# zhan-xu/MoRig

Measured on AMD Instinct MI355X. Metric: meshes/sec jointnet_motion forward, 4 k-vert synthetic, higher is better.
Workload: dtype f32 (split-fp16: 3x f16 MFMA, f32 accumulate); 1 GPU; jointnet_motion(num_keyframes=5, attn) eval forward, B=64 x 4096-vertex synthetic meshes/GPU, BASELINE.json configs[1]; step=COO->CSR prep + forward, meshes_per_gpu=64, global_batch=64, vertices_per_mesh=4096, parallelism=mesh-sharded dp1, guard_read=deferred, geo_graph=device

## Files before the change

morig_amd/csrc/common.h:

```cpp
#pragma once
#include <hip/hip_runtime.h>
#include <stdint.h>
#include <string.h>
#include "../../include/morig_hip.h"
#include "ragged_core.h"

namespace morig {

enum Kind : int {
    K_GEMM_BN128 = 0, K_GEMM_BN64, K_GEMM_BN32, K_GEMM_POOL,
    K_EDGE_H16, K_EDGE_H32, K_EDGE_H64, K_EDGE_H128, K_EDGE_H256,
    K_CSR, K_COPY, K_ROWNORM, K_ATTN, K_MISC,
    K_FPS, K_BALL, K_POINTCONV, K_KNN_INTERP, K_COSINE_NN,
    K_GEMM16_BN128, K_GEMM16_BN64, K_GEMM16_BN32, K_GEMM16_POOL,
    K_EDGE16_H32, K_EDGE16_H64, K_EDGE16_H128, K_EDGE16_H256, K_POINTCONV16, K_GEMM16_DMA,
    K_COSINE_KNN, K_FLOW_VOTE, K_JOINTS,
    K_GEMM16_DMAP, K_GEMM16_DMA128, K_EDGE16_H256_PP, K_EDGE16_H128_WS, K_EDGE16_PC, K_GEOGRAPH, K_EDGE16_X3, K_EDGE_X3, K_EDGE16_X3P, K_EDGE16_H128_RL,
    K_LOSS_NCE_FWD, K_LOSS_NCE_BWD, K_LOSS_MULTIPOS, K_LOSS_CHAMFER, K_LOSS_REDUCE,
    K_LOSS_LOGRATIO, K_LOSS_SKIN_CE,
    K_METRICS,
    K_RIG_ASSEMBLE, K_RIG_ENTRIES,
    K_RANSAC_VOTE, K_RANSAC_FIT, K_RANSAC_APPLY, K_KMEANS,
    K_MESH_PREP, K_VOXEL_SURFACE, K_VOXEL_FILL,
    K_POSE_PREP, K_POSE_SKIN, K_POSE_ERRORS,
    K_SCAN_RASTER, K_SCAN,
    K_SIMPLIFY_KEYS, K_SIMPLIFY_QUADRICS,
    K_COUNT
};
static_assert(K_COUNT <= MORIG_PROF_KINDS, "raise MORIG_PROF_KINDS");

void set_hip_error(hipError_t e);
struct ProfScope {
    ProfScope(int kind, hipStream_t s, double flops, double bytes);
    ~ProfScope();
    int slot; hipStream_t stream; ProfScope* outer;
};
void prof_retag(int kind);

inline int check_hip(hipError_t e) {
    if (e == hipSuccess) return MORIG_OK;
    set_hip_error(e);
    return MORIG_E_HIP;
}
#define MORIG_HIP_TRY(expr) do { hipError_t _e = (expr); if (_e != hipSuccess) { ::morig::set_hip_error(_e); return MORIG_E_HIP; } } while (0)
#define MORIG_LAUNCH_CHECK() MORIG_HIP_TRY(hipGetLastError())

struct EdgePcParams {
    int H;
    const float* W; int ldw;
    const float* bias; const float* scale; const float* shift;
    const float* A; int lda; const float* B; int ldb;
    const int* rowptr; const int* srcS; const int* dstS; int n_nodes; int rep_in; int rep_out; int tiles_per_rep;
    int replicas;
    float* Y; int ldy;
    int y16;
    int run;
    int* ovf;
    int quad;
    int min4;
    unsigned long long* trace;
    int dbg;
};
struct GemmDmaParams {
    int M, N, K;
    const float* X; int ldx;
    const float* Xt; int ldt; int tail_rows; int tail_chunks;
    const float* W; int ldw;
    const float* bias; const float* scale; const float* shift; int relu;
    const float* rowbias; int ld_rowbias; const int* seg;
    float* Y; int ldy; int y16;
    float* pool; int ld_pool;
    int tiles_n;
    int* ovf;
    int dbg;
    unsigned long long* trace;
};
int launch_edge_pc(const EdgePcParams& p, int nblocks, hipStream_t s);
void set_reserved_cus(int n);
int reserved_cus();
int launch_edge_pp(const EdgePcParams& p, int nblocks, hipStream_t s);
int launch_edge_ws(const EdgePcParams& p, int nblocks, hipStream_t s);
int launch_edge_rl(const EdgePcParams& p, int ntiles64, hipStream_t s);
int launch_gemm16_dma(const GemmDmaParams& p, int tiles_m128, hipStream_t s);
struct EdgeX3Params {
    const float* X; int ldx;
    const float* W1a; const float* W1b; const float* b1;
    const float* A; int lda; const float* B; int ldb;
    const float* W2s; int ldw;
    const float* bias; const float* scale; const float* shift;
    const int* rowptr; const int* srcS; const int* dstS; int n_nodes; int cap;
    int rep_in, rep_out, replicas;
    float* Y; int ldy;
    int* ovf;
};

int launch_edge_x3(const EdgeX3Params& p, int n_tiles_cap, hipStream_t s);
int launch_gemm16_dmap(const GemmDmaParams& p, hipStream_t s);
bool few_rows_gemm_takes(int M, int N, int K, int ldx, int ldw);
int launch_few_rows_gemm(const float* X, int ldx, int M, const float* W, int ldw, int N, int K, const float* bias, const float* scale,
                         const float* shift, int relu, float* Y, int ldy, hipStream_t s);

static_assert(sizeof(morig_gemm_args) >= MORIG_GEMM_ARGS_V3_SIZE && sizeof(morig_edgeconv_args) >= MORIG_EDGECONV_ARGS_V3_SIZE &&
              sizeof(morig_edgeconv_x3_args) >= MORIG_EDGECONV_X3_ARGS_V3_SIZE && sizeof(morig_segmax_args) >= MORIG_SEGMAX_ARGS_V3_SIZE &&
              sizeof(morig_pointconv_args) >= MORIG_POINTCONV_ARGS_V3_SIZE, "argument structs only grow");
static_assert(sizeof(morig_edgeconv_args) == MORIG_EDGECONV_ARGS_SIZE && sizeof(morig_edgeconv_x3_args) == MORIG_EDGECONV_X3_ARGS_SIZE,
              "include/morig_hip.h states the current sizes");
template <class T> static inline bool take_args(const T* a, T& mine, uint32_t v3_size) {
    if (!a) return false;
    const uint32_t n = a->struct_size;
    if (n < v3_size || n > 1024u || (n & 7u)) return false;
    memset(&mine, 0, sizeof(T));
    memcpy(&mine, a, n < sizeof(T) ? n : sizeof(T));
    mine.struct_size = (uint32_t)sizeof(T);
    return true;
}

static inline int cdiv(long a, long b) { return (int)((a + b - 1) / b); }

__device__ __forceinline__ void atomic_max_f32(float* addr, float v) {
    if (v == 0.0f) v = 0.0f;
    if (v >= 0.0f) atomicMax(reinterpret_cast<int*>(addr), __float_as_int(v));
    else           atomicMin(reinterpret_cast<unsigned int*>(addr), __float_as_uint(v));
}

__device__ __forceinline__ int xcd_remap(int b, int n) {
    const int q = n >> 3, r = n & 7, x = b & 7, i = b >> 3;
    return (x < r ? x * (q + 1) : r * (q + 1) + (x - r) * q) + i;
}

inline int stats_slab_rows(int rows_cap, int cols) {
    const int groups = (cols + 63) / 64;
    int slabs = 1024 / (groups > 0 ? groups : 1);
    if (slabs < 64) slabs = 64;
    int r = ((rows_cap > 0 ? rows_cap : 1) + slabs - 1) / slabs;
    r = (r + 3) & ~3;
    return r < 256 ? 256 : r;
}

#ifdef __HIPCC__
__device__ inline void split_pair_f16(float v0, float v1, float& hi, float& lo) {
    typedef __fp16 split_h2 __attribute__((ext_vector_type(2)));
    const split_h2 h = __builtin_amdgcn_cvt_pkrtz(v0, v1);
    hi = __builtin_bit_cast(float, h);
#ifdef MORIG_SPLIT_C_FORM
    split_h2 l;
    l[0] = (__fp16)(v0 - (float)h[0]); l[1] = (__fp16)(v1 - (float)h[1]);
    lo = __builtin_bit_cast(float, l);
#else
    asm("v_fma_mixlo_f16 %0, %1, 1.0, -%2 op_sel_hi:[0,0,1]" : "=v"(lo) : "v"(v0), "v"(hi));
    asm("v_fma_mixhi_f16 %0, %1, 1.0, -%2 op_sel:[0,0,1] op_sel_hi:[0,0,1]" : "+v"(lo) : "v"(v1), "v"(hi));
#endif
}
#endif

#ifdef __HIPCC__
__device__ inline void split_pair_bf16(float v0, float v1, float& hi, float& lo) {
    typedef __bf16 split_b2 __attribute__((ext_vector_type(2)));
    const split_b2 h = {(__bf16)v0, (__bf16)v1};
    const unsigned hb = __builtin_bit_cast(unsigned, h);
    hi = __builtin_bit_cast(float, h);
    const float r0 = v0 - __uint_as_float(hb << 16), r1 = v1 - __uint_as_float(hb & 0xffff0000u);
    const split_b2 l = {(__bf16)r0, (__bf16)r1};
    lo = __builtin_bit_cast(float, l);
}
#endif

#ifdef __HIPCC__
__device__ inline void split_pair_bf16_rem(float v0, float v1, float& hi, float& r0, float& r1) {
    typedef __bf16 split_b2 __attribute__((ext_vector_type(2)));
    const split_b2 h = {(__bf16)v0, (__bf16)v1};
    const unsigned hb = __builtin_bit_cast(unsigned, h);
    hi = __builtin_bit_cast(float, h);
    r0 = v0 - __uint_as_float(hb << 16);
    r1 = v1 - __uint_as_float(hb & 0xffff0000u);
}
#endif

template <int V> struct VecF { float v[V]; };
#ifdef __HIPCC__
template <int V> __device__ inline VecF<V> ldv(const float* p) {
    VecF<V> r;
    if constexpr (V == 4) { const float4 t = *reinterpret_cast<const float4*>(p); r.v[0] = t.x; r.v[1] = t.y; r.v[2] = t.z; r.v[3] = t.w; }
    else r.v[0] = *p;
    return r;
}
template <int V> __device__ inline void stv(float* p, const VecF<V>& r) {
    if constexpr (V == 4) *reinterpret_cast<float4*>(p) = make_float4(r.v[0], r.v[1], r.v[2], r.v[3]);
    else *p = r.v[0];
}
#endif
static inline bool vec4_ptr(const void* p, long ld) { return (reinterpret_cast<uintptr_t>(p) & 15) == 0 && (ld & 3) == 0; }

#ifdef __HIPCC__
__device__ inline void stats_block_store(const double (&acc)[2][4], int quads, int RL, int q, int rl, int c0, int cols, int slab,
                                         double* __restrict__ part) {
    __shared__ double sh[2 * 1024];
    const int gc = quads * 4;
    if (rl < RL) {
#pragma unroll
        for (int k = 0; k < 2; ++k)
#pragma unroll
            for (int j = 0; j < 4; ++j) sh[(k * gc + q * 4 + j) * RL + rl] = acc[k][j];
    }
    __syncthreads();
    const int t = threadIdx.x;
    if (t < 2 * gc) {
        const int k = t / gc, col = t - k * gc;
        double s = 0.0;
        for (int i = 0; i < RL; ++i) s += sh[(k * gc + col) * RL + i];
        if (c0 + col < cols) part[((size_t)slab * 2 + k) * cols + c0 + col] = s;
    }
}

constexpr int STATS_FC = 4;
__device__ inline void stats_final_sums(const double* __restrict__ part, int slabs, int cols, int c, double& s, double& q) {
    const int sl = threadIdx.x / STATS_FC, l = threadIdx.x % STATS_FC;
    constexpr int LANES = 256 / STATS_FC;
    s = 0.0; q = 0.0;
    if (c < cols)
        for (int b = sl; b < slabs; b += LANES) { s += part[((size_t)b * 2 + 0) * cols + c]; q += part[((size_t)b * 2 + 1) * cols + c]; }
    __shared__ double sh[2][LANES][STATS_FC];
    sh[0][sl][l] = s; sh[1][sl][l] = q;
    __syncthreads();
    for (int h = LANES / 2; h > 0; h >>= 1) {
        if (sl < h) { sh[0][sl][l] += sh[0][sl + h][l]; sh[1][sl][l] += sh[1][sl + h][l]; }
        __syncthreads();
    }
    s = sh[0][0][l]; q = sh[1][0][l];
}

__device__ __forceinline__ double block_sum256(double s, double* sh) {
    sh[threadIdx.x] = s;
    __syncthreads();
    for (int h = 128; h > 0; h >>= 1) {
        if ((int)threadIdx.x < h) sh[threadIdx.x] += sh[threadIdx.x + h];
        __syncthreads();
    }
    const double r = sh[0];
    __syncthreads();
    return r;
}
#endif

}
```

morig_amd/csrc/gemm_dma.hip:

```cpp
#include "common.h"
#include "epilogue_store.h"
#include <stdlib.h>
#include <stdlib.h>

namespace morig {

typedef float f32x16 __attribute__((ext_vector_type(16)));
typedef _Float16 f16x8 __attribute__((ext_vector_type(8)));
typedef __attribute__((address_space(3))) void lds_void_t;
typedef __attribute__((address_space(1))) const void glb_void_t;

template <int BM, int BN, int NT, int DMA_NS, bool TR = false, bool TAIL = false>
__global__ __launch_bounds__((BM / 64) * (BN / (32 * NT)) * 64) void gemm16_dma_kernel(const GemmDmaParams p) {
    constexpr int MT = 2;
    constexpr int WNW = BN / (32 * NT);
    constexpr int NW = (BM / 64) * WNW;
    constexpr int DMA_STAGE = (BM + BN) * 128;
    constexpr int XJ = BM / 8 / NW, WJ = BN / 8 / NW;
    constexpr int PER_CHUNK = XJ + WJ;
    constexpr int TBYTES = NW * EpilogueTile<NT>::FLOATS * 4;
    constexpr int RING = DMA_NS * DMA_STAGE;
    constexpr int SM0 = (TR || RING > TBYTES) ? RING : TBYTES;
    constexpr int PANEL = TR ? 3 * BN * 4 : 0;
    __shared__ __attribute__((aligned(128))) char smem[SM0 + BM * 4 + PANEL];
    int* sseg = reinterpret_cast<int*>(smem + SM0);
    float* pan = reinterpret_cast<float*>(smem + SM0 + BM * 4);

    const int tid = threadIdx.x, lane = tid & 63, wave = tid >> 6;
    const int l31 = lane & 31, hi = lane >> 5;
    const int wm = wave / WNW, wn = wave % WNW;
    const int lin = xcd_remap(blockIdx.x, gridDim.x);
    const int tn = lin % p.tiles_n, tm = lin / p.tiles_n;
    const int row0 = tm * BM;

#ifdef MORIG_DMA_TRACE
#define DMA_TS(k) do { if ((int)blockIdx.x == (int)(gridDim.x / 2 + 8) && lane == 0) p.trace[(k) * 8 + wave] = __builtin_readcyclecounter(); } while (0)
#else
#define DMA_TS(k) do { } while (0)
#endif
    DMA_TS(0);
    if (!TR && p.seg != nullptr && tid < BM) sseg[tid] = (row0 + tid < p.M) ? p.seg[row0 + tid] : 0;
    float pv_b = 0.f, pv_s = 1.f, pv_t = 0.f;
    bool rb_slow = false;
    if constexpr (TR) {
        if (tid < BN) {
            const int col = tn * BN + tid;
            if (p.bias) pv_b = p.bias[col];
            if (p.scale) { pv_s = p.scale[col]; pv_t = p.shift[col]; }
        }
        if (p.rowbias != nullptr) {
            const int s0 = p.seg[row0], s1 = p.seg[min(row0 + BM, p.M) - 1];
            rb_slow = s0 != s1;
            if (!rb_slow && tid < BN) pv_b += p.rowbias[(size_t)s0 * p.ld_rowbias + tn * BN + tid];
        }
    }

    unsigned ox[XJ], ow[WJ];
    const int rsub = lane >> 3;
    const int pslot = lane & 7;
    const char* xbase = reinterpret_cast<const char*>(p.X + (size_t)row0 * p.ldx);
    const char* wbase = reinterpret_cast<const char*>(p.W + (size_t)(tn * BN) * p.ldw);
#pragma unroll
    for (int j = 0; j < XJ; ++j) {
        const int r = (wave * XJ + j) * 8 + rsub;
        const int lslot = pslot ^ ((r >> 1) & 7);
        int xr = r; if (row0 + xr >= p.M) xr = p.M - 1 - row0;
        ox[j] = ((unsigned)xr * (unsigned)p.ldx + 4u * lslot) * 4u;
    }
#pragma unroll
    for (int j = 0; j < WJ; ++j) {
        const int r = (wave * WJ + j) * 8 + rsub;
        ow[j] = ((unsigned)r * (unsigned)p.ldw + 4u * (pslot ^ ((r >> 1) & 7))) * 4u;
    }
    const int nchunk = (p.K + 31) / 32;
    unsigned ot[TAIL ? XJ : 1];
    const int c_tail = TAIL ? nchunk - p.tail_chunks : nchunk;
    const char* tbase = reinterpret_cast<const char*>(p.Xt);
    if constexpr (TAIL) {
#pragma unroll
        for (int j = 0; j < XJ; ++j) {
            const int r = (wave * XJ + j) * 8 + rsub;
            int gr = row0 + r; if (gr >= p.M) gr = p.M - 1;
            ot[j] = ((unsigned)(gr % p.tail_rows) * (unsigned)p.ldt + 4u * (unsigned)(pslot ^ ((r >> 1) & 7))) * 4u;
        }
    }
    auto x_src = [&](int c, int j) __attribute__((always_inline)) -> const char* {
        unsigned o = ox[j];
        const char* b = xbase + c * 128;
        if constexpr (TAIL) { if (c >= c_tail) { o = ot[j]; b = tbase + (c - c_tail) * 128; } }
        asm volatile("" : "+v"(o));
        return b + o;
    };
    auto issue_x = [&](int c) {
        char* st = smem + (c % DMA_NS) * DMA_STAGE;
#pragma unroll
        for (int j = 0; j < XJ; ++j)
            __builtin_amdgcn_global_load_lds((glb_void_t*)x_src(c, j), (lds_void_t*)(st + (wave * XJ + j) * 1024), 16, 0, 0);
    };
    auto issue_w = [&](int c) {
        char* st = smem + (c % DMA_NS) * DMA_STAGE;
#pragma unroll
        for (int j = 0; j < WJ; ++j) {
            unsigned o = ow[j];
            asm volatile("" : "+v"(o));
            __builtin_amdgcn_global_load_lds((glb_void_t*)(wbase + c * 128 + o), (lds_void_t*)(st + BM * 128 + (wave * WJ + j) * 1024), 16, 0, 0);
        }
    };
    auto issue = [&](int c) { issue_x(c); issue_w(c); };

    f32x16 acc[MT][NT];
#pragma unroll
    for (int mt = 0; mt < MT; ++mt)
#pragma unroll
        for (int nt = 0; nt < NT; ++nt)
#pragma unroll
            for (int r = 0; r < 16; ++r) acc[mt][nt][r] = 0.f;

#pragma unroll
    for (int c = 0; c < DMA_NS - 1; ++c) if (c < nchunk) issue(c);
    if constexpr (TR) { if (tid < BN) { pan[tid] = pv_b; pan[BN + tid] = pv_s; pan[2 * BN + tid] = pv_t; } }

    const int x7 = (l31 >> 1) & 7;
    const int aoff = (wm * 64 + l31) * 128, boff = BM * 128 + (wn * NT * 32 + l31) * 128;
    struct Frag { f16x8 ah[MT], al[MT], bh[NT], bl[NT]; };
    auto load_frag = [&](Frag& f, int c, int s2) {
        const char* st = smem + (c % DMA_NS) * DMA_STAGE;
        const int sh = ((2 * s2 + hi) ^ x7) * 16, sl = ((4 + 2 * s2 + hi) ^ x7) * 16;
#pragma unroll
        for (int mt = 0; mt < MT; ++mt) {
            f.ah[mt] = *reinterpret_cast<const f16x8*>(st + aoff + mt * 32 * 128 + sh);
            f.al[mt] = *reinterpret_cast<const f16x8*>(st + aoff + mt * 32 * 128 + sl);
        }
#pragma unroll
        for (int nt = 0; nt < NT; ++nt) {
            f.bh[nt] = *reinterpret_cast<const f16x8*>(st + boff + nt * 32 * 128 + sh);
            f.bl[nt] = *reinterpret_cast<const f16x8*>(st + boff + nt * 32 * 128 + sl);
        }
    };
    auto mm = [&](const f16x8& x, const f16x8& w, f32x16& c) __attribute__((always_inline)) {
        if constexpr (TR) c = __builtin_amdgcn_mfma_f32_32x32x16_f16(w, x, c, 0, 0, 0);
        else              c = __builtin_amdgcn_mfma_f32_32x32x16_f16(x, w, c, 0, 0, 0);
    };
    auto mma = [&](const Frag& f) {
#pragma unroll
        for (int mt = 0; mt < MT; ++mt)
#pragma unroll
            for (int nt = 0; nt < NT; ++nt) {
                mm(f.al[mt], f.bh[nt], acc[mt][nt]);
#ifndef MORIG_2MFMA
                mm(f.ah[mt], f.bl[nt], acc[mt][nt]);
#endif
                mm(f.ah[mt], f.bh[nt], acc[mt][nt]);
            }
    };
    auto wait_chunk = [&](int c) {
        int younger = nchunk - 1 - c;
        if (younger > DMA_NS - 2) younger = DMA_NS - 2;
        static_assert(DMA_NS >= 2 && DMA_NS <= 4, "ring depth");
        if (younger == 2) asm volatile("s_waitcnt vmcnt(%0)" ::"n"(2 * PER_CHUNK) : "memory");
        else if (younger == 1) asm volatile("s_waitcnt vmcnt(%0)" ::"n"(PER_CHUNK) : "memory");
        else asm volatile("s_waitcnt vmcnt(0)" ::: "memory");
    };
    auto mma_pair = [&](const Frag& f, int mt, int nt0) __attribute__((always_inline)) {
        mm(f.al[mt], f.bh[nt0],     acc[mt][nt0]);
        mm(f.al[mt], f.bh[nt0 + 1], acc[mt][nt0 + 1]);
#ifndef MORIG_2MFMA
        mm(f.ah[mt], f.bl[nt0],     acc[mt][nt0]);
        mm(f.ah[mt], f.bl[nt0 + 1], acc[mt][nt0 + 1]);
#endif
        mm(f.ah[mt], f.bh[nt0],     acc[mt][nt0]);
        mm(f.ah[mt], f.bh[nt0 + 1], acc[mt][nt0 + 1]);
    };
    auto issue_one = [&](int c, int j) __attribute__((always_inline)) {
        char* st = smem + (c % DMA_NS) * DMA_STAGE;
        if (j < XJ) {
            __builtin_amdgcn_global_load_lds((glb_void_t*)x_src(c, j), (lds_void_t*)(st + (wave * XJ + j) * 1024), 16, 0, 0);
        } else {
            unsigned o = ow[j - XJ];
            asm volatile("" : "+v"(o));
            __builtin_amdgcn_global_load_lds((glb_void_t*)(wbase + c * 128 + o), (lds_void_t*)(st + BM * 128 + (wave * WJ + j - XJ) * 1024), 16, 0, 0);
        }
    };
    Frag f0, f1;
    wait_chunk(0);
    if constexpr (TR) asm volatile("s_waitcnt lgkmcnt(0)" ::: "memory");
    __builtin_amdgcn_s_barrier();
    if (DMA_NS - 1 < nchunk) issue(DMA_NS - 1);
    if constexpr (TR) {
        typedef float pf32x4 __attribute__((ext_vector_type(4)));
#pragma unroll
        for (int nt = 0; nt < NT; ++nt)
#pragma unroll
            for (int g4 = 0; g4 < 4; ++g4) {
                const pf32x4 b4 = *reinterpret_cast<const pf32x4*>(pan + wn * NT * 32 + nt * 32 + 8 * g4 + 4 * hi);
#pragma unroll
                for (int mt = 0; mt < MT; ++mt)
#pragma unroll
                    for (int q = 0; q < 4; ++q) acc[mt][nt][4 * g4 + q] = b4[q];
            }
    }
    load_frag(f0, 0, 0);
#ifdef MORIG_DMA_BURST
    constexpr bool SPREAD = false;
#else
    constexpr bool SPREAD = (NT == 4 && MT == 2 && PER_CHUNK == 8);
#endif
    for (int c = 0; c < nchunk; ++c) {
        load_frag(f1, c, 1);
        mma(f0);
        const bool more = c + 1 < nchunk;
        const bool dma = c + DMA_NS < nchunk;
        if (more) {
            wait_chunk(c + 1);
            asm volatile("s_waitcnt lgkmcnt(0)" ::: "memory");
            __builtin_amdgcn_s_barrier();
            if constexpr (!SPREAD) { if (dma) issue(c + DMA_NS); }
            load_frag(f0, c + 1, 0);
        }
        if constexpr (SPREAD) {
            const bool go = more && dma;
            mma_pair(f1, 0, 0); __builtin_amdgcn_sched_barrier(0);
            if (go) { issue_one(c + DMA_NS, 0); issue_one(c + DMA_NS, 1); }
            __builtin_amdgcn_sched_barrier(0);
            mma_pair(f1, 0, 2); __builtin_amdgcn_sched_barrier(0);
            if (go) { issue_one(c + DMA_NS, 2); issue_one(c + DMA_NS, 3); }
            __builtin_amdgcn_sched_barrier(0);
            mma_pair(f1, 1, 0); __builtin_amdgcn_sched_barrier(0);
            if (go) { issue_one(c + DMA_NS, 4); issue_one(c + DMA_NS, 5); }
            __builtin_amdgcn_sched_barrier(0);
            mma_pair(f1, 1, 2); __builtin_amdgcn_sched_barrier(0);
            if (go) { issue_one(c + DMA_NS, 6); issue_one(c + DMA_NS, 7); }
            __builtin_amdgcn_sched_barrier(0);
        } else {
            mma(f1);
        }
    }

    DMA_TS(1);
    const int colw0 = tn * BN + wn * NT * 32;
    if (!TR && p.pool != nullptr) {
        const int rfirst = row0 + wm * 64;
        if (rfirst >= p.M) return;
        const int rlast = min(rfirst + 63, p.M - 1);
        const int s0 = p.seg[rfirst];
        const bool uni = s0 == p.seg[rlast];
#pragma unroll
        for (int nt = 0; nt < NT; ++nt) {
            const int col = colw0 + nt * 32 + l31;
            const bool cok = col < p.N;
            const float b = (p.bias && cok) ? p.bias[col] : 0.f;
            const float sc = (p.scale && cok) ? p.scale[col] : 1.f;
            const float shf = (p.shift && cok) ? p.shift[col] : 0.f;
            float m = -INFINITY;
#pragma unroll
            for (int mt = 0; mt < MT; ++mt)
#pragma unroll
                for (int r = 0; r < 16; ++r) {
                    const int row = rfirst + mt * 32 + (r & 3) + 8 * (r >> 2) + 4 * hi;
                    float v = acc[mt][nt][r] + b;
                    if (p.relu) v = v > 0.f ? v : 0.f;
                    v = v * sc + shf;
                    if (row < p.M) {
                        if (uni) m = fmaxf(m, v);
                        else if (cok) atomic_max_f32(p.pool + (size_t)p.seg[row] * p.ld_pool + col, v);
                    }
                }
            if (uni) {
                m = fmaxf(m, __shfl_xor(m, 32, 64));
                if (hi == 0 && cok && m > -INFINITY) atomic_max_f32(p.pool + (size_t)s0 * p.ld_pool + col, m);
            }
        }
        return;
    }
    if constexpr (TR) {
        if (p.dbg & 1) { if (acc[0][0][0] == 12345.678f) p.Y[0] = 1.f; return; }
        DMA_TS(2);
        store_tile_regs<MT, NT>(p, acc, p.scale ? pan + BN : nullptr, pan + 2 * BN, wm * 64, row0, p.M, colw0, wn * NT * 32, lane, rb_slow);
        DMA_TS(3);
        return;
    }
    __syncthreads();
    if (p.dbg & 1) { if (acc[0][0][0] == 12345.678f) p.Y[0] = 1.f; return; }
    DMA_TS(2);
    store_tile_transposed<MT, NT, true>(p, acc, reinterpret_cast<float*>(smem) + wave * EpilogueTile<NT>::FLOATS, sseg,
                                        wm * 64, row0, p.M, colw0, lane);
    DMA_TS(3);
#ifdef MORIG_DMA_TRACE
    asm volatile("s_waitcnt vmcnt(0)" ::: "memory");
    DMA_TS(4);
#endif
}

int launch_gemm16_dma(const GemmDmaParams& p0, int tiles_m128, hipStream_t s) {
    GemmDmaParams p = p0;
    static const int dbg = [] { const char* e = getenv("MORIG_DEBUG_FLAGS"); return e ? atoi(e) : 0; }();
    p.dbg = dbg;
    static const int mode = [] { const char* e = getenv("MORIG_DMA_TILE"); return e ? atoi(e) : 256; }();
    static const int persist = [] { const char* e = getenv("MORIG_DMA_PERSIST"); return e ? (e[0] == '0' ? 0 : 2) : 1; }();
    const bool deep_wide = p.pool != nullptr || (p.K >= 768 && p.N >= 1024);
    const bool vec_ok = p.pool != nullptr ||
                        ((reinterpret_cast<uintptr_t>(p.Y) & 15) == 0 && (p.ldy & 3) == 0 &&
                         (!p.rowbias || ((reinterpret_cast<uintptr_t>(p.rowbias) & 15) == 0 && (p.ld_rowbias & 3) == 0)));
    if (p.Xt && !(mode == 256 && p.N % 256 == 0 && !p.pool)) return MORIG_E_UNSUPPORTED;
    static const int small_tiles = [] { const char* e = getenv("MORIG_DMA_SMALL_TILES"); return e ? atoi(e) : 256; }();
    const bool few_tiles = !p.Xt && p.N % 256 == 0 && (long)cdiv(p.M, 256) * (p.N / 256) <= small_tiles;
    if (!few_tiles && !p.Xt && mode == 256 && p.N % 256 == 0 && p.K > 32 && vec_ok && (persist == 2 || (persist == 1 && deep_wide))) {
        if (!p.pool) prof_retag(K_GEMM16_DMAP);
        return launch_gemm16_dmap(p0, s);
    }
    if (mode == 256 && p.N % 256 == 0 && !few_tiles) {
        p.tiles_n = p.N / 256;
        const int nb = cdiv(p.M, 256) * p.tiles_n;
#ifdef MORIG_DMA_TRACE
        static unsigned long long* trace_buf = [] { void* b = nullptr; return hipMalloc(&b, 64 * 8) == hipSuccess ? (unsigned long long*)b : nullptr; }();
        p.trace = trace_buf;
#endif
        static const bool want_tr = [] { const char* e = getenv("MORIG_GEMM_TR"); return !(e && e[0] == '0'); }();
        const bool tr = want_tr && !p.pool && (reinterpret_cast<uintptr_t>(p.Y) & 15) == 0 && (p.ldy & 3) == 0 &&
                        (!p.rowbias || ((reinterpret_cast<uintptr_t>(p.rowbias) & 15) == 0 && (p.ld_rowbias & 3) == 0));
        static const int shortk = [] { const char* e = getenv("MORIG_DMA_SHORTK"); return e ? atoi(e) : 0; }();
        if (tr && !p.Xt && shortk > 0 && p.K <= shortk && p.N % 128 == 0) {
            p.tiles_n = p.N / 128;
            const int nb128 = cdiv(p.M, 128) * p.tiles_n;
            prof_retag(K_GEMM16_DMA128);
            hipLaunchKernelGGL((gemm16_dma_kernel<128, 128, 2, 2, true>), dim3(nb128), dim3(256), 0, s, p);
            MORIG_LAUNCH_CHECK();
            return MORIG_OK;
        }
        if (p.Xt && !tr) return MORIG_E_UNSUPPORTED;
        if (p.Xt)    hipLaunchKernelGGL((gemm16_dma_kernel<256, 256, 4, 2, true, true>), dim3(nb), dim3(512), 0, s, p);
        else if (tr) hipLaunchKernelGGL((gemm16_dma_kernel<256, 256, 4, 2, true>), dim3(nb), dim3(512), 0, s, p);
        else         hipLaunchKernelGGL((gemm16_dma_kernel<256, 256, 4, 2, false>), dim3(nb), dim3(512), 0, s, p);
#ifdef MORIG_DMA_TRACE
        {
            unsigned long long h[64];
            if (hipStreamSynchronize(s) == hipSuccess && hipMemcpy(h, p.trace, sizeof(h), hipMemcpyDeviceToHost) == hipSuccess) {
                fprintf(stderr, "DMA_TRACE K=%d N=%d:", p.K, p.N);
                for (int w = 0; w < 8; w += 3) { fprintf(stderr, " w%d", w); for (int q = 1; q < 5; ++q) fprintf(stderr, " %lld", (long long)(h[q * 8 + w] - h[(q - 1) * 8 + w])); }
                fprintf(stderr, "\n");
            }
        }
#endif
    } else {
        p.tiles_n = cdiv(p.N, 128);
        prof_retag(K_GEMM16_DMA128);
        hipLaunchKernelGGL((gemm16_dma_kernel<128, 128, 2, 2, false>), dim3(tiles_m128 * p.tiles_n), dim3(256), 0, s, p);
    }
    MORIG_LAUNCH_CHECK();
    return MORIG_OK;
}

}
```

morig_amd/csrc/gemm_dmap.hip:

```cpp
#include "common.h"
#include "epilogue_store.h"
#include <atomic>
#include <stdlib.h>
#include <type_traits>

namespace morig {

typedef float f32x16 __attribute__((ext_vector_type(16)));
typedef _Float16 f16x8 __attribute__((ext_vector_type(8)));
typedef __attribute__((address_space(3))) void lds_void_t;
typedef __attribute__((address_space(1))) const void glb_void_t;

struct GemmDmaHot { int M, K, ldx, ldw, tiles_n; const float* X; const float* W; const int* seg; };
typedef __attribute__((address_space(4))) const GemmDmaParams* kernarg_params_t;
template <bool POOL>
__global__ __launch_bounds__(512) void gemm16_dmap_kernel(const GemmDmaParams) {
#if defined(__HIP_DEVICE_COMPILE__)
    kernarg_params_t q = (kernarg_params_t)__builtin_amdgcn_kernarg_segment_ptr();
    asm volatile("" : "+s"(q));
    const GemmDmaHot p = {q->M, q->K, q->ldx, q->ldw, q->tiles_n, q->X, q->W, q->seg};
    constexpr int BM = 256, BN = 256, NT = 4, MT = 2;
    constexpr int WNW = BN / (32 * NT);
    constexpr int NW = (BM / 64) * WNW;
    constexpr int STAGE = (BM + BN) * 128;
    constexpr int XJ = BM / 8 / NW, WJ = BN / 8 / NW;
    constexpr int PANEL = 3 * BN;
    __shared__ __attribute__((aligned(128))) char smem[2 * STAGE + (POOL ? 0 : 2 * PANEL * 4)];
    float* pan = reinterpret_cast<float*>(smem + 2 * STAGE);

    const int tid = threadIdx.x, lane = tid & 63, wave = tid >> 6;
    const int l31 = lane & 31, hi = lane >> 5;
    const int wm = wave / WNW, wn = wave % WNW;

    const int tiles_m = (p.M + BM - 1) / BM;
    const int T = tiles_m * p.tiles_n;
    const int xcd = blockIdx.x & 7, bi = blockIdx.x >> 3, nbx = gridDim.x >> 3;
    const int t_lo = (int)((long long)T * xcd / 8), t_hi = (int)((long long)T * (xcd + 1) / 8);
    const int n_my = (t_hi - t_lo - bi + nbx - 1) / nbx;
    if (n_my <= 0) return;

    const int nchunk = (p.K + 31) / 32;
    const int rsub = lane >> 3, pslot = lane & 7;
    unsigned ow[WJ];
#pragma unroll
    for (int j = 0; j < WJ; ++j) {
        const int r = (wave * WJ + j) * 8 + rsub;
        ow[j] = ((unsigned)r * (unsigned)p.ldw + 4u * (pslot ^ ((r >> 1) & 7))) * 4u;
    }
    auto x_offset = [&](int j, int row0) __attribute__((always_inline)) {
        const int r = (wave * XJ + j) * 8 + rsub;
        int xr = r; if (row0 + xr >= p.M) xr = p.M - 1 - row0;
        return ((unsigned)xr * (unsigned)p.ldx + 4u * (pslot ^ ((r >> 1) & 7))) * 4u;
    };
    auto dma_x = [&](const char* xb, unsigned o, int c, int stage, int j) __attribute__((always_inline)) {
#ifdef DMAP_ABL_HOT
        xb = reinterpret_cast<const char*>(p.X); c = 0;
#endif
        asm volatile("" : "+v"(o));
        __builtin_amdgcn_global_load_lds((glb_void_t*)(xb + c * 128 + o), (lds_void_t*)(smem + stage * STAGE + (wave * XJ + j) * 1024), 16, 0, 0);
    };
    auto dma_w = [&](const char* wb, int c, int stage, int j) __attribute__((always_inline)) {
#ifdef DMAP_ABL_HOT
        wb = reinterpret_cast<const char*>(p.W); c = 0;
#endif
        unsigned o = ow[j];
        asm volatile("" : "+v"(o));
        __builtin_amdgcn_global_load_lds((glb_void_t*)(wb + c * 128 + o), (lds_void_t*)(smem + stage * STAGE + BM * 128 + (wave * WJ + j) * 1024), 16, 0, 0);
    };

    const int x7 = (l31 >> 1) & 7;
    const int aoff = (wm * 64 + l31) * 128, boff = BM * 128 + (wn * NT * 32 + l31) * 128;
    struct Frag { f16x8 ah[MT], al[MT], bh[NT], bl[NT]; };
    auto load_frag = [&](Frag& f, int stage, int s2) __attribute__((always_inline)) {
        const char* st = smem + stage * STAGE;
        const int sh = ((2 * s2 + hi) ^ x7) * 16, sl = ((4 + 2 * s2 + hi) ^ x7) * 16;
#pragma unroll
        for (int mt = 0; mt < MT; ++mt) {
            f.ah[mt] = *reinterpret_cast<const f16x8*>(st + aoff + mt * 32 * 128 + sh);
            f.al[mt] = *reinterpret_cast<const f16x8*>(st + aoff + mt * 32 * 128 + sl);
        }
#pragma unroll
        for (int nt = 0; nt < NT; ++nt) {
            f.bh[nt] = *reinterpret_cast<const f16x8*>(st + boff + nt * 32 * 128 + sh);
            f.bl[nt] = *reinterpret_cast<const f16x8*>(st + boff + nt * 32 * 128 + sl);
        }
    };
    f32x16 acc[MT][NT];
    auto mm = [&](const f16x8& x, const f16x8& w, f32x16& c) __attribute__((always_inline)) {
        if constexpr (POOL) c = __builtin_amdgcn_mfma_f32_32x32x16_f16(x, w, c, 0, 0, 0);
        else                c = __builtin_amdgcn_mfma_f32_32x32x16_f16(w, x, c, 0, 0, 0);
    };
    auto mma = [&](const Frag& f) __attribute__((always_inline)) {
#pragma unroll
        for (int mt = 0; mt < MT; ++mt)
#pragma unroll
            for (int nt = 0; nt < NT; ++nt) {
                mm(f.al[mt], f.bh[nt], acc[mt][nt]);
                mm(f.ah[mt], f.bl[nt], acc[mt][nt]);
                mm(f.ah[mt], f.bh[nt], acc[mt][nt]);
            }
    };
    auto mma_pair = [&](const Frag& f, int mt, int nt0) __attribute__((always_inline)) {
        mm(f.al[mt], f.bh[nt0],     acc[mt][nt0]);
        mm(f.al[mt], f.bh[nt0 + 1], acc[mt][nt0 + 1]);
        mm(f.ah[mt], f.bl[nt0],     acc[mt][nt0]);
        mm(f.ah[mt], f.bl[nt0 + 1], acc[mt][nt0 + 1]);
        mm(f.ah[mt], f.bh[nt0],     acc[mt][nt0]);
        mm(f.ah[mt], f.bh[nt0 + 1], acc[mt][nt0 + 1]);
    };
    float pv0 = 0.f, pv1 = 0.f;
    auto panel_fetch = [&](int plin, bool& slow) __attribute__((always_inline)) {
        asm volatile("" : "+s"(q));
        const float* bias = q->bias; const float* scale = q->scale; const float* shift = q->shift;
        const float* rowbias = q->rowbias; const int* seg = q->seg;
        const int col = (plin % p.tiles_n) * BN + (tid & (BN - 1));
        slow = false;
        pv0 = 0.f; pv1 = 0.f;
        if (tid < BN) {
            if (bias) pv0 = bias[col];
        } else if (scale) { pv0 = scale[col]; pv1 = shift[col]; }
        if (rowbias != nullptr) {
            const int prow0 = (plin / p.tiles_n) * BM;
            const int s0 = seg[prow0], s1 = seg[min(prow0 + BM, p.M) - 1];
            slow = s0 != s1;
            if (!slow && tid < BN) pv1 = rowbias[(size_t)s0 * q->ld_rowbias + col];
        }
    };
    auto panel_write = [&](int par) __attribute__((always_inline)) {
        float* pn = pan + par * PANEL;
        if (tid < BN) pn[tid] = pv0 + pv1;
        else { pn[BN + (tid - BN)] = pv0; pn[2 * BN + (tid - BN)] = pv1; }
    };

    unsigned ox[XJ];
    Frag f0, f1;
    auto chunk_iter = [&](int st, auto morec, auto goc, const char* xb, const char* wb, int cc, bool reclamp, int nrow0)
                          __attribute__((always_inline)) {
#ifdef DMAP_ABL_NODMA
        constexpr bool more = decltype(morec)::value != 0, go = false;
#else
        constexpr bool more = decltype(morec)::value != 0, go = decltype(goc)::value != 0;
#endif
#ifdef DMAP_ABL_NOFRAG
        asm volatile("" : "+v"(f1.ah[0]), "+v"(f1.al[0]), "+v"(f1.ah[1]), "+v"(f1.al[1]));
        asm volatile("" : "+v"(f1.bh[0]), "+v"(f1.bl[0]), "+v"(f1.bh[1]), "+v"(f1.bl[1]), "+v"(f1.bh[2]), "+v"(f1.bl[2]), "+v"(f1.bh[3]), "+v"(f1.bl[3]));
#else
        load_frag(f1, st, 1);
#endif
        mma(f0);
        if constexpr (more) {
#ifndef DMAP_ABL_NOWAIT
            asm volatile("s_waitcnt vmcnt(0)" ::: "memory");
#endif
            asm volatile("s_waitcnt lgkmcnt(0)" ::: "memory");
            __builtin_amdgcn_s_barrier();
#ifdef DMAP_ABL_NOFRAG
            asm volatile("" : "+v"(f0.ah[0]), "+v"(f0.al[0]), "+v"(f0.ah[1]), "+v"(f0.al[1]));
            asm volatile("" : "+v"(f0.bh[0]), "+v"(f0.bl[0]), "+v"(f0.bh[1]), "+v"(f0.bl[1]), "+v"(f0.bh[2]), "+v"(f0.bl[2]), "+v"(f0.bh[3]), "+v"(f0.bl[3]));
#else
            load_frag(f0, st ^ 1, 0);
#endif
        }
        unsigned o0 = ox[0], o1 = ox[1], o2 = ox[2], o3 = ox[3];
        if (go && reclamp) { o0 = x_offset(0, nrow0); o1 = x_offset(1, nrow0); o2 = x_offset(2, nrow0); o3 = x_offset(3, nrow0); }
        mma_pair(f1, 0, 0); __builtin_amdgcn_sched_barrier(0);
        if constexpr (go) { dma_x(xb, o0, cc, st, 0); dma_x(xb, o1, cc, st, 1); }
        __builtin_amdgcn_sched_barrier(0);
        mma_pair(f1, 0, 2); __builtin_amdgcn_sched_barrier(0);
        if constexpr (go) { dma_x(xb, o2, cc, st, 2); dma_x(xb, o3, cc, st, 3); }
        __builtin_amdgcn_sched_barrier(0);
        mma_pair(f1, 1, 0); __builtin_amdgcn_sched_barrier(0);
        if constexpr (go) { dma_w(wb, cc, st, 0); dma_w(wb, cc, st, 1); }
        __builtin_amdgcn_sched_barrier(0);
        mma_pair(f1, 1, 2); __builtin_amdgcn_sched_barrier(0);
        if constexpr (go) { dma_w(wb, cc, st, 2); dma_w(wb, cc, st, 3); }
        __builtin_amdgcn_sched_barrier(0);
    };
    typedef std::integral_constant<int, 1> Yes;
    typedef std::integral_constant<int, 0> No;

    int lin = t_lo + bi;
    int g = 0;
    {
        const int row0 = (lin / p.tiles_n) * BM;
        const char* xbase = reinterpret_cast<const char*>(p.X + (size_t)row0 * p.ldx);
        const char* wbase = reinterpret_cast<const char*>(p.W + (size_t)((lin % p.tiles_n) * BN) * p.ldw);
#pragma unroll
        for (int j = 0; j < XJ; ++j) dma_x(xbase, x_offset(j, row0), 0, 0, j);
#pragma unroll
        for (int j = 0; j < WJ; ++j) dma_w(wbase, 0, 0, j);
    }
    bool slow_cur = false, slow_next = false;
    if constexpr (!POOL) { panel_fetch(lin, slow_cur); }
    asm volatile("s_waitcnt vmcnt(0)" ::: "memory");
    if constexpr (!POOL) { panel_write(0); asm volatile("s_waitcnt lgkmcnt(0)" ::: "memory"); }

#pragma unroll 1
    for (int jt = 0; jt < n_my; ++jt) {
        const int tn = lin % p.tiles_n, row0 = (lin / p.tiles_n) * BM;
        const char* xbase = reinterpret_cast<const char*>(p.X + (size_t)row0 * p.ldx);
        const char* wbase = reinterpret_cast<const char*>(p.W + (size_t)(tn * BN) * p.ldw);
#pragma unroll
        for (int j = 0; j < XJ; ++j) ox[j] = x_offset(j, row0);

        __builtin_amdgcn_s_barrier();
#pragma unroll
        for (int j = 0; j < XJ; ++j) dma_x(xbase, ox[j], 1, (g + 1) & 1, j);
#pragma unroll
        for (int j = 0; j < WJ; ++j) dma_w(wbase, 1, (g + 1) & 1, j);
        if constexpr (POOL) {
#pragma unroll
            for (int mt = 0; mt < MT; ++mt)
#pragma unroll
                for (int nt = 0; nt < NT; ++nt)
#pragma unroll
                    for (int r = 0; r < 16; ++r) acc[mt][nt][r] = 0.f;
        } else {
            typedef float pf32x4 __attribute__((ext_vector_type(4)));
            const float* pn = pan + (jt & 1) * PANEL + wn * NT * 32 + 4 * hi;
#pragma unroll
            for (int nt = 0; nt < NT; ++nt)
#pragma unroll
                for (int g4 = 0; g4 < 4; ++g4) {
                    const pf32x4 b4 = *reinterpret_cast<const pf32x4*>(pn + nt * 32 + 8 * g4);
#pragma unroll
                    for (int mt = 0; mt < MT; ++mt)
#pragma unroll
                        for (int qq = 0; qq < 4; ++qq) acc[mt][nt][4 * g4 + qq] = b4[qq];
                }
        }
        load_frag(f0, g & 1, 0);

#pragma unroll 1
        for (int c = 0; c + 2 < nchunk; ++c) chunk_iter((g + c) & 1, Yes{}, Yes{}, xbase, wbase, c + 2, false, 0);
        {
            const int nlin = jt + 1 < n_my ? lin + nbx : lin;
            const int nrow0 = (nlin / p.tiles_n) * BM;
            const char* nxbase = reinterpret_cast<const char*>(p.X + (size_t)nrow0 * p.ldx);
            const char* nwbase = reinterpret_cast<const char*>(p.W + (size_t)((nlin % p.tiles_n) * BN) * p.ldw);
            if constexpr (!POOL) panel_fetch(nlin, slow_next);
            chunk_iter((g + nchunk - 2) & 1, Yes{}, Yes{}, nxbase, nwbase, 0, true, nrow0);
            chunk_iter((g + nchunk - 1) & 1, No{}, No{}, nxbase, nwbase, 0, false, 0);
            lin = nlin;
        }

        asm volatile("s_waitcnt vmcnt(0) lgkmcnt(0)" ::: "memory");
        const int colw0 = tn * BN + wn * NT * 32;
        if constexpr (POOL) {
            asm volatile("" : "+s"(q));
            GemmDmaParams pe;
            pe.M = q->M; pe.N = q->N; pe.bias = q->bias; pe.scale = q->scale; pe.shift = q->shift; pe.relu = q->relu; pe.seg = q->seg;
            pe.pool = q->pool; pe.ld_pool = q->ld_pool;
            const int rfirst = row0 + wm * 64;
            if (rfirst < pe.M) {
                const int rlast = min(rfirst + 63, pe.M - 1);
                const int s0 = pe.seg[rfirst];
                const bool uni = s0 == pe.seg[rlast];
#pragma unroll
                for (int nt = 0; nt < NT; ++nt) {
                    const int col = colw0 + nt * 32 + l31;
                    const bool cok = col < pe.N;
                    const float b = (pe.bias && cok) ? pe.bias[col] : 0.f;
                    const float sc = (pe.scale && cok) ? pe.scale[col] : 1.f;
                    const float shf = (pe.shift && cok) ? pe.shift[col] : 0.f;
                    float m = -INFINITY;
#pragma unroll
                    for (int mt = 0; mt < MT; ++mt)
#pragma unroll
                        for (int r = 0; r < 16; ++r) {
                            const int row = rfirst + mt * 32 + (r & 3) + 8 * (r >> 2) + 4 * hi;
                            float v = acc[mt][nt][r] + b;
                            if (pe.relu) v = v > 0.f ? v : 0.f;
                            v = v * sc + shf;
                            if (row < pe.M) {
                                if (uni) m = fmaxf(m, v);
                                else if (cok) atomic_max_f32(pe.pool + (size_t)pe.seg[row] * pe.ld_pool + col, v);
                            }
                        }
                    if (uni) {
                        m = fmaxf(m, __shfl_xor(m, 32, 64));
                        if (hi == 0 && cok && m > -INFINITY) atomic_max_f32(pe.pool + (size_t)s0 * pe.ld_pool + col, m);
                    }
                }
            }
        } else {
            panel_write((jt + 1) & 1);
            asm volatile("" : "+s"(q));
            GemmDmaParams pe;
            pe.M = q->M; pe.N = q->N; pe.scale = q->scale; pe.relu = q->relu;
            pe.rowbias = q->rowbias; pe.ld_rowbias = q->ld_rowbias; pe.seg = q->seg;
            pe.Y = q->Y; pe.ldy = q->ldy; pe.y16 = q->y16; pe.ovf = q->ovf; pe.dbg = q->dbg;
            const float* pn = pan + (jt & 1) * PANEL;
            if (!(pe.dbg & 1))
                store_tile_regs<MT, NT>(pe, acc, pe.scale ? pn + BN : nullptr, pn + 2 * BN, wm * 64, row0, pe.M, colw0, wn * NT * 32, lane,
                                        slow_cur);
            slow_cur = slow_next;
        }
        g += nchunk;
    }
    asm volatile("s_waitcnt vmcnt(0)" ::: "memory");
#endif
}

static int cu_count() {
    static std::atomic<int> cache[64];
    int dev = 0;
    if (hipGetDevice(&dev) != hipSuccess || dev < 0 || dev >= 64) return 256;
    int n = cache[dev].load();
    if (n == 0) {
        if (hipDeviceGetAttribute(&n, hipDeviceAttributeMultiprocessorCount, dev) != hipSuccess || n <= 0) n = 256;
        cache[dev].store(n);
    }
    return n;
}

int launch_gemm16_dmap(const GemmDmaParams& p0, hipStream_t s) {
    GemmDmaParams p = p0;
    static const int dbg = [] { const char* e = getenv("MORIG_DEBUG_FLAGS"); return e ? atoi(e) : 0; }();
    p.dbg = dbg;
    p.tiles_n = p.N / 256;
    const int T = cdiv(p.M, 256) * p.tiles_n;
    int ncu = cu_count();
    ncu = ncu > 8 ? (ncu / 8) * 8 : 8;
    int avail = ncu - ((reserved_cus() + 7) / 8) * 8;
    if (avail < 8) avail = 8;
    const int grid = T < avail ? ((T + 7) / 8) * 8 : avail;
    if (p.pool) hipLaunchKernelGGL(gemm16_dmap_kernel<true>, dim3(grid), dim3(512), 0, s, p);
    else        hipLaunchKernelGGL(gemm16_dmap_kernel<false>, dim3(grid), dim3(512), 0, s, p);
    MORIG_LAUNCH_CHECK();
    return MORIG_OK;
}

}
```

Measured before the change: 1438 meshes/s.

## Schedule pooled GEMM tiles as row runs and defer segment-max atomics across tiles

In the pooled (segment max) GEMM path, each workgroup now walks runs of consecutive row tiles in the same column block rather than strided tiles. Per-column max and min are kept in LDS across the tiles of a run and flushed with one atomic max per segment when the segment changes or the run ends. This cuts global atomic traffic and the per-tile vmcnt drains. It also applies bias, relu and scale once at flush time, using the min when the scale is negative. The costs are extra LDS, more complex tile scheduling with a host-chosen run length, and possible load imbalance across workgroups.

```diff
diff --git a/morig_amd/csrc/common.h b/morig_amd/csrc/common.h
--- a/morig_amd/csrc/common.h
+++ b/morig_amd/csrc/common.h
@@ -71,6 +71,7 @@
     float* Y; int ldy; int y16;
     float* pool; int ld_pool;
     int tiles_n;
+    int run;
     int* ovf;
     int dbg;
     unsigned long long* trace;
diff --git a/morig_amd/csrc/gemm_dma.hip b/morig_amd/csrc/gemm_dma.hip
--- a/morig_amd/csrc/gemm_dma.hip
+++ b/morig_amd/csrc/gemm_dma.hip
@@ -1,5 +1,6 @@
 #include "common.h"
 #include "epilogue_store.h"
+#include "pool_epilogue.h"
 #include <stdlib.h>
 #include <stdlib.h>
 
@@ -241,35 +242,7 @@
     if (!TR && p.pool != nullptr) {
         const int rfirst = row0 + wm * 64;
         if (rfirst >= p.M) return;
-        const int rlast = min(rfirst + 63, p.M - 1);
-        const int s0 = p.seg[rfirst];
-        const bool uni = s0 == p.seg[rlast];
-#pragma unroll
-        for (int nt = 0; nt < NT; ++nt) {
-            const int col = colw0 + nt * 32 + l31;
-            const bool cok = col < p.N;
-            const float b = (p.bias && cok) ? p.bias[col] : 0.f;
-            const float sc = (p.scale && cok) ? p.scale[col] : 1.f;
-            const float shf = (p.shift && cok) ? p.shift[col] : 0.f;
-            float m = -INFINITY;
-#pragma unroll
-            for (int mt = 0; mt < MT; ++mt)
-#pragma unroll
-                for (int r = 0; r < 16; ++r) {
-                    const int row = rfirst + mt * 32 + (r & 3) + 8 * (r >> 2) + 4 * hi;
-                    float v = acc[mt][nt][r] + b;
-                    if (p.relu) v = v > 0.f ? v : 0.f;
-                    v = v * sc + shf;
-                    if (row < p.M) {
-                        if (uni) m = fmaxf(m, v);
-                        else if (cok) atomic_max_f32(p.pool + (size_t)p.seg[row] * p.ld_pool + col, v);
-                    }
-                }
-            if (uni) {
-                m = fmaxf(m, __shfl_xor(m, 32, 64));
-                if (hi == 0 && cok && m > -INFINITY) atomic_max_f32(p.pool + (size_t)s0 * p.ld_pool + col, m);
-            }
-        }
+        pool_tile<MT, NT>(p, acc, rfirst, colw0, lane);
         return;
     }
     if constexpr (TR) {
diff --git a/morig_amd/csrc/gemm_dmap.hip b/morig_amd/csrc/gemm_dmap.hip
--- a/morig_amd/csrc/gemm_dmap.hip
+++ b/morig_amd/csrc/gemm_dmap.hip
@@ -1,5 +1,7 @@
 #include "common.h"
 #include "epilogue_store.h"
+#include "pool_epilogue.h"
+#include "pool_runs.h"
 #include <atomic>
 #include <stdlib.h>
 #include <type_traits>
@@ -25,7 +27,8 @@
     constexpr int STAGE = (BM + BN) * 128;
     constexpr int XJ = BM / 8 / NW, WJ = BN / 8 / NW;
     constexpr int PANEL = 3 * BN;
-    __shared__ __attribute__((aligned(128))) char smem[2 * STAGE + (POOL ? 0 : 2 * PANEL * 4)];
+    constexpr int PAIR = 2 * NT * 64;
+    __shared__ __attribute__((aligned(128))) char smem[2 * STAGE + (POOL ? NW * PAIR * 4 : 2 * PANEL * 4)];
     float* pan = reinterpret_cast<float*>(smem + 2 * STAGE);
 
     const int tid = threadIdx.x, lane = tid & 63, wave = tid >> 6;
@@ -36,7 +39,15 @@
     const int T = tiles_m * p.tiles_n;
     const int xcd = blockIdx.x & 7, bi = blockIdx.x >> 3, nbx = gridDim.x >> 3;
     const int t_lo = (int)((long long)T * xcd / 8), t_hi = (int)((long long)T * (xcd + 1) / 8);
-    const int n_my = (t_hi - t_lo - bi + nbx - 1) / nbx;
+    int run_u = 0, run_left = 0;
+    int n_my;
+    if constexpr (POOL) {
+        int u_end, u_stride;
+        n_my = pool_wg_tiles(tiles_m, p.tiles_n, q->run, (int)gridDim.x, (int)blockIdx.x);
+        pool_wg_runs(pool_run_units(tiles_m, p.tiles_n, q->run), (int)gridDim.x, (int)blockIdx.x, run_u, u_end, u_stride);
+    } else {
+        n_my = (t_hi - t_lo - bi + nbx - 1) / nbx;
+    }
     if (n_my <= 0) return;
 
     const int nchunk = (p.K + 31) / 32;
@@ -180,6 +191,20 @@
     typedef std::integral_constant<int, 0> No;
 
     int lin = t_lo + bi;
+    if constexpr (POOL) {
+        lin = pool_run_first_tile(run_u, p.tiles_n, q->run);
+        run_left = pool_run_count(run_u, tiles_m, p.tiles_n, q->run) - 1;
+    }
+    typedef float pf32x4 __attribute__((ext_vector_type(4)));
+    static_assert(NT == 4 && PAIR == 2 * 4 * 64, "the pair is kept as two 16-byte vectors per thread");
+    auto pair_ptr = [&](int t) __attribute__((always_inline)) { return reinterpret_cast<pf32x4*>(smem + 2 * STAGE) + t; };
+    int rseg = -1;
+    bool drained = true;
+    const int wave_s = __builtin_amdgcn_readfirstlane(wave);
+    if constexpr (POOL) {
+        pair_ptr(tid)[0] = pf32x4{-INFINITY, -INFINITY, -INFINITY, -INFINITY};
+        pair_ptr(tid)[512] = pf32x4{INFINITY, INFINITY, INFINITY, INFINITY};
+    }
     int g = 0;
     {
         const int row0 = (lin / p.tiles_n) * BM;
@@ -202,7 +227,13 @@
         const char* wbase = reinterpret_cast<const char*>(p.W + (size_t)(tn * BN) * p.ldw);
 #pragma unroll
         for (int j = 0; j < XJ; ++j) ox[j] = x_offset(j, row0);
-
+        bool run_end = true;
+
+        if constexpr (POOL) {
+            if (!drained) asm volatile("s_waitcnt vmcnt(0)" ::: "memory");
+            asm volatile("s_waitcnt lgkmcnt(0)" ::: "memory");
+            drained = false;
+        }
         __builtin_amdgcn_s_barrier();
 #pragma unroll
         for (int j = 0; j < XJ; ++j) dma_x(xbase, ox[j], 1, (g + 1) & 1, j);
@@ -234,7 +265,18 @@
 #pragma unroll 1
         for (int c = 0; c + 2 < nchunk; ++c) chunk_iter((g + c) & 1, Yes{}, Yes{}, xbase, wbase, c + 2, false, 0);
         {
-            const int nlin = jt + 1 < n_my ? lin + nbx : lin;
+            int nlin = jt + 1 < n_my ? lin + nbx : lin;
+            if constexpr (POOL) {
+                run_end = run_left == 0;
+                if (!run_end) { nlin = lin + p.tiles_n; --run_left; }
+                else if (jt + 1 < n_my) {
+                    asm volatile("" : "+s"(q));
+                    const int R = q->run;
+                    run_u += nbx;
+                    nlin = pool_run_first_tile(run_u, p.tiles_n, R);
+                    run_left = pool_run_count(run_u, tiles_m, p.tiles_n, R) - 1;
+                }
+            }
             const int nrow0 = (nlin / p.tiles_n) * BM;
             const char* nxbase = reinterpret_cast<const char*>(p.X + (size_t)nrow0 * p.ldx);
             const char* nwbase = reinterpret_cast<const char*>(p.W + (size_t)((nlin % p.tiles_n) * BN) * p.ldw);
@@ -244,45 +286,51 @@
             lin = nlin;
         }
 
-        asm volatile("s_waitcnt vmcnt(0) lgkmcnt(0)" ::: "memory");
+        if constexpr (!POOL) asm volatile("s_waitcnt vmcnt(0) lgkmcnt(0)" ::: "memory");
         const int colw0 = tn * BN + wn * NT * 32;
         if constexpr (POOL) {
-            asm volatile("" : "+s"(q));
-            GemmDmaParams pe;
-            pe.M = q->M; pe.N = q->N; pe.bias = q->bias; pe.scale = q->scale; pe.shift = q->shift; pe.relu = q->relu; pe.seg = q->seg;
-            pe.pool = q->pool; pe.ld_pool = q->ld_pool;
-            const int rfirst = row0 + wm * 64;
-            if (rfirst < pe.M) {
-                const int rlast = min(rfirst + 63, pe.M - 1);
-                const int s0 = pe.seg[rfirst];
-                const bool uni = s0 == pe.seg[rlast];
-#pragma unroll
-                for (int nt = 0; nt < NT; ++nt) {
-                    const int col = colw0 + nt * 32 + l31;
-                    const bool cok = col < pe.N;
-                    const float b = (pe.bias && cok) ? pe.bias[col] : 0.f;
-                    const float sc = (pe.scale && cok) ? pe.scale[col] : 1.f;
-                    const float shf = (pe.shift && cok) ? pe.shift[col] : 0.f;
-                    float m = -INFINITY;
-#pragma unroll
-                    for (int mt = 0; mt < MT; ++mt)
-#pragma unroll
-                        for (int r = 0; r < 16; ++r) {
-                            const int row = rfirst + mt * 32 + (r & 3) + 8 * (r >> 2) + 4 * hi;
-                            float v = acc[mt][nt][r] + b;
-                            if (pe.relu) v = v > 0.f ? v : 0.f;
-                            v = v * sc + shf;
-                            if (row < pe.M) {
-                                if (uni) m = fmaxf(m, v);
-                                else if (cok) atomic_max_f32(pe.pool + (size_t)pe.seg[row] * pe.ld_pool + col, v);
-                            }
-                        }
-                    if (uni) {
-                        m = fmaxf(m, __shfl_xor(m, 32, 64));
-                        if (hi == 0 && cok && m > -INFINITY) atomic_max_f32(pe.pool + (size_t)s0 * pe.ld_pool + col, m);
-                    }
-                }
+            const int elane = __builtin_amdgcn_mbcnt_hi(~0u, __builtin_amdgcn_mbcnt_lo(~0u, 0u)), ewave = wave_s;
+            const int te = ewave * 64 + elane;
+            const int ecolw0 = tn * BN + (ewave % WNW) * NT * 32;
+            const int rfirst = row0 + (ewave / WNW) * 64;
+            pf32x4* const pair_mx = pair_ptr(te);
+            pf32x4* const pair_mn = pair_mx + 512;
+            auto drain = [&]() __attribute__((always_inline)) {
+                if (!drained) { asm volatile("s_waitcnt vmcnt(0)" ::: "memory"); drained = true; }
+            };
+            auto load_pe = [&](GemmDmaParams& pe) __attribute__((always_inline)) {
+                asm volatile("" : "+s"(q));
+                pe.M = q->M; pe.N = q->N; pe.bias = q->bias; pe.scale = q->scale; pe.shift = q->shift; pe.relu = q->relu; pe.seg = q->seg;
+                pe.pool = q->pool; pe.ld_pool = q->ld_pool;
+            };
+            auto flush = [&]() __attribute__((always_inline)) {
+                drain();
+                GemmDmaParams pe;
+                load_pe(pe);
+                const pf32x4 vx = *pair_mx, vn = *pair_mn;
+                const float mx[NT] = {vx[0], vx[1], vx[2], vx[3]}, mn[NT] = {vn[0], vn[1], vn[2], vn[3]};
+                pool_flush<NT>(pe, rseg, ecolw0, elane, mx, mn);
+                *pair_mx = pf32x4{-INFINITY, -INFINITY, -INFINITY, -INFINITY};
+                *pair_mn = pf32x4{INFINITY, INFINITY, INFINITY, INFINITY};
+                rseg = -1;
+            };
+            int s0 = -1;
+            const bool whole = pool_slab_is_uniform(p, rfirst, s0);
+            if (rseg >= 0 && !(whole && s0 == rseg)) flush();
+            if (whole) {
+                const pf32x4 vx = *pair_mx, vn = *pair_mn;
+                float mx[NT] = {vx[0], vx[1], vx[2], vx[3]}, mn[NT] = {vn[0], vn[1], vn[2], vn[3]};
+                pool_reduce_rows<MT, NT>(acc, mx, mn);
+                *pair_mx = pf32x4{mx[0], mx[1], mx[2], mx[3]};
+                *pair_mn = pf32x4{mn[0], mn[1], mn[2], mn[3]};
+                rseg = s0;
+            } else if (rfirst < p.M) {
+                drain();
+                GemmDmaParams pe;
+                load_pe(pe);
+                pool_tile_per_element<MT, NT>(pe, acc, rfirst, ecolw0, elane);
             }
+            if (run_end && rseg >= 0) flush();
         } else {
             panel_write((jt + 1) & 1);
             asm volatile("" : "+s"(q));
@@ -325,6 +373,10 @@
     int avail = ncu - ((reserved_cus() + 7) / 8) * 8;
     if (avail < 8) avail = 8;
     const int grid = T < avail ? ((T + 7) / 8) * 8 : avail;
+    static const int run_env = [] { const char* e = getenv("MORIG_POOL_RUN"); const int v = e ? atoi(e) : 0; return v < 0 ? 0 : (v > 256 ? 256 : v); }();
+    if (!p.pool) p.run = 1;
+    else if (run_env > 0) p.run = pool_run_length(cdiv(p.M, 256), p.tiles_n, 0, run_env);
+    else p.run = pool_run_length(cdiv(p.M, 256), p.tiles_n, grid, 16);
     if (p.pool) hipLaunchKernelGGL(gemm16_dmap_kernel<true>, dim3(grid), dim3(512), 0, s, p);
     else        hipLaunchKernelGGL(gemm16_dmap_kernel<false>, dim3(grid), dim3(512), 0, s, p);
     MORIG_LAUNCH_CHECK();
diff --git a/morig_amd/csrc/pool_epilogue.h b/morig_amd/csrc/pool_epilogue.h
--- /dev/null
+++ b/morig_amd/csrc/pool_epilogue.h
@@ -0,0 +1,107 @@
+#pragma once
+#include "common.h"
+
+namespace morig {
+
+typedef float pool_f32x16 __attribute__((ext_vector_type(16)));
+
+__device__ __forceinline__ float pool_transform(float a, float b, float sc, float shf, int relu) {
+    float v = a + b;
+    if (relu) v = v > 0.f ? v : 0.f;
+    v = v * sc + shf;
+    return v;
+}
+
+template <int NT> __device__ __forceinline__ void pool_pair_identity(float (&mx)[NT], float (&mn)[NT]) {
+#pragma unroll
+    for (int nt = 0; nt < NT; ++nt) { mx[nt] = -INFINITY; mn[nt] = INFINITY; }
+}
+
+template <int MT, int NT>
+__device__ __forceinline__ void pool_reduce_rows(const pool_f32x16 (&acc)[MT][NT], float (&mx)[NT], float (&mn)[NT]) {
+#pragma unroll
+    for (int nt = 0; nt < NT; ++nt) {
+        float a = mx[nt], i = mn[nt];
+#pragma unroll
+        for (int mt = 0; mt < MT; ++mt)
+#pragma unroll
+            for (int r = 0; r < 16; r += 2) {
+                const float x = acc[mt][nt][r], y = acc[mt][nt][r + 1];
+                asm("v_max3_f32 %0, %1, %2, %0" : "+v"(a) : "v"(x), "v"(y));
+                asm("v_min3_f32 %0, %1, %2, %0" : "+v"(i) : "v"(x), "v"(y));
+            }
+        mx[nt] = a; mn[nt] = i;
+    }
+}
+
+template <int NT, class P>
+__device__ __forceinline__ void pool_flush(const P& p, int sg, int colw0, int lane, const float (&mx)[NT], const float (&mn)[NT]) {
+    const int l31 = lane & 31, hi = lane >> 5;
+#pragma unroll
+    for (int nt = 0; nt < NT; ++nt) {
+        const int col = colw0 + nt * 32 + l31;
+        const bool cok = col < p.N;
+        const float b = (p.bias && cok) ? p.bias[col] : 0.f;
+        const float sc = (p.scale && cok) ? p.scale[col] : 1.f;
+        const float shf = (p.shift && cok) ? p.shift[col] : 0.f;
+        const float a = fmaxf(mx[nt], __shfl_xor(mx[nt], 32, 64));
+        const float i = fminf(mn[nt], __shfl_xor(mn[nt], 32, 64));
+        const float m = pool_transform(sc < 0.f ? i : a, b, sc, shf, p.relu);
+        if (hi == 0 && cok && m > -INFINITY) atomic_max_f32(p.pool + (size_t)sg * p.ld_pool + col, m);
+    }
+}
+
+template <int MT, int NT, class P>
+__device__ __forceinline__ void pool_tile_per_element(const P& p, const pool_f32x16 (&acc)[MT][NT], int rfirst, int colw0, int lane) {
+    const int l31 = lane & 31, hi = lane >> 5;
+    const int rlast = min(rfirst + 63, p.M - 1);
+    const int s0 = p.seg[rfirst];
+    const bool uni = s0 == p.seg[rlast];
+#pragma unroll
+    for (int nt = 0; nt < NT; ++nt) {
+        const int col = colw0 + nt * 32 + l31;
+        const bool cok = col < p.N;
+        const float b = (p.bias && cok) ? p.bias[col] : 0.f;
+        const float sc = (p.scale && cok) ? p.scale[col] : 1.f;
+        const float shf = (p.shift && cok) ? p.shift[col] : 0.f;
+        float m = -INFINITY;
+#pragma unroll
+        for (int mt = 0; mt < MT; ++mt)
+#pragma unroll
+            for (int r = 0; r < 16; ++r) {
+                const int row = rfirst + mt * 32 + (r & 3) + 8 * (r >> 2) + 4 * hi;
+                const float v = pool_transform(acc[mt][nt][r], b, sc, shf, p.relu);
+                if (row < p.M) {
+                    if (uni) m = fmaxf(m, v);
+                    else if (cok) atomic_max_f32(p.pool + (size_t)p.seg[row] * p.ld_pool + col, v);
+                }
+            }
+        if (uni) {
+            m = fmaxf(m, __shfl_xor(m, 32, 64));
+            if (hi == 0 && cok && m > -INFINITY) atomic_max_f32(p.pool + (size_t)s0 * p.ld_pool + col, m);
+        }
+    }
+}
+
+template <class P> __device__ __forceinline__ bool pool_slab_is_uniform(const P& p, int rfirst, int& sg) {
+    typedef __attribute__((address_space(4))) const int* const_int_ptr;
+    if (rfirst + 63 >= p.M) return false;
+    const_int_ptr seg = (const_int_ptr)p.seg;
+    sg = seg[rfirst];
+    return sg == seg[rfirst + 63];
+}
+
+template <int MT, int NT, class P>
+__device__ __forceinline__ void pool_tile(const P& p, const pool_f32x16 (&acc)[MT][NT], int rfirst, int colw0, int lane) {
+    int sg = 0;
+    if (pool_slab_is_uniform(p, rfirst, sg)) {
+        float mx[NT], mn[NT];
+        pool_pair_identity<NT>(mx, mn);
+        pool_reduce_rows<MT, NT>(acc, mx, mn);
+        pool_flush<NT>(p, sg, colw0, lane, mx, mn);
+    } else {
+        pool_tile_per_element<MT, NT>(p, acc, rfirst, colw0, lane);
+    }
+}
+
+}
diff --git a/morig_amd/csrc/pool_runs.h b/morig_amd/csrc/pool_runs.h
--- /dev/null
+++ b/morig_amd/csrc/pool_runs.h
@@ -0,0 +1,47 @@
+#pragma once
+
+#if defined(__HIPCC__) || defined(__CUDACC__)
+#define MORIG_POOL_HD __host__ __device__ inline
+#else
+#define MORIG_POOL_HD inline
+#endif
+
+namespace morig {
+
+MORIG_POOL_HD int pool_run_units(int tiles_m, int tiles_n, int R) { return ((tiles_m + R - 1) / R) * tiles_n; }
+
+MORIG_POOL_HD void pool_wg_runs(int units, int grid, int block, int& first, int& end, int& stride) {
+    const int xcd = block & 7, bi = block >> 3;
+    stride = grid >> 3;
+    first = (int)((long long)units * xcd / 8) + bi;
+    end = (int)((long long)units * (xcd + 1) / 8);
+}
+
+MORIG_POOL_HD int pool_run_col_block(int u, int tiles_n) { return u % tiles_n; }
+MORIG_POOL_HD int pool_run_first_row_tile(int u, int tiles_n, int R) { return (u / tiles_n) * R; }
+MORIG_POOL_HD int pool_run_count(int u, int tiles_m, int tiles_n, int R) {
+    const int left = tiles_m - pool_run_first_row_tile(u, tiles_n, R);
+    return left < R ? left : R;
+}
+MORIG_POOL_HD int pool_run_first_tile(int u, int tiles_n, int R) {
+    return pool_run_first_row_tile(u, tiles_n, R) * tiles_n + pool_run_col_block(u, tiles_n);
+}
+
+MORIG_POOL_HD int pool_wg_tiles(int tiles_m, int tiles_n, int R, int grid, int block) {
+    int first, end, stride, n = 0;
+    pool_wg_runs(pool_run_units(tiles_m, tiles_n, R), grid, block, first, end, stride);
+    if (R == 1) return first < end ? (end - first + stride - 1) / stride : 0;
+    for (int u = first; u < end; u += stride) n += pool_run_count(u, tiles_m, tiles_n, R);
+    return n;
+}
+
+MORIG_POOL_HD int pool_run_length(int tiles_m, int tiles_n, int grid, int r_max) {
+    int R = 1;
+    while (R * 2 <= r_max) R *= 2;
+    const int nbx = grid >> 3;
+    if (nbx <= 0) return R;
+    while (R > 1 && (pool_run_units(tiles_m, tiles_n, R) / 8) / nbx < 2) R >>= 1;
+    return R;
+}
+
+}
```

Result: faster. 1458 meshes/s (median of 6 runs) (+1.4%).
